# Sunshine-718/AlphaZero-AL

Hardware: AMD Instinct MI355X
Metric: self-play positions/sec (Connect4 n_playout=200, batch=8192 games/GPU, vl_batch=4) (higher is better)
Workload: dtype f32; 1 GPU; Connect4 self-play, n_playout=200, 8192 games/GPU, vl_batch=4, evaluator=cnn; c_base=1000, use_symmetry=True, lead_in_plies=12, streams_per_gpu=1, parallelism=independent game shards x1

## Files before the change

alphazero-al_amd/csrc/nn_conv.hip:

```cpp
#include <cstdio>
#include <cstdlib>

#include "az_nn.h"
#include "nn_common.h"

namespace {

constexpr int CELLS = 42, COLS = 7;
constexpr int PCOLS = 8, PCELLS = 72;
constexpr int TS = 4;
constexpr int COUT = 64;
constexpr int CELLB = 128;

template <int N>
__device__ __forceinline__ void stage_sample(const void *base, uint32_t voff, uint32_t lds_off, uint64_t last_mask)
{
    uint32_t keep;
    uint64_t ex;
    if constexpr (N == 6)
        asm volatile("s_mov_b32 %0, m0\n\ts_mov_b32 m0, %4\n\ts_nop 2\n\t"
                     "global_load_lds_dwordx4 %2, %3\n\t"
                     "global_load_lds_dwordx4 %2, %3 offset:1024\n\t"
                     "global_load_lds_dwordx4 %2, %3 offset:2048\n\t"
                     "global_load_lds_dwordx4 %2, %3 offset:3072\n\t"
                     "s_mov_b32 m0, %6\n\ts_nop 0\n\t"
                     "global_load_lds_dwordx4 %5, %3\n\t"
                     "s_and_saveexec_b64 %1, %7\n\t"
                     "global_load_lds_dwordx4 %5, %3 offset:1024\n\t"
                     "s_mov_b64 exec, %1\n\ts_mov_b32 m0, %0"
                     : "=&s"(keep), "=&s"(ex)
                     : "v"(voff), "s"(base), "s"(lds_off), "v"(voff + 4096), "s"(lds_off + 4096), "s"(last_mask)
                     : "memory", "scc");
    else
        asm volatile("s_mov_b32 %0, m0\n\ts_mov_b32 m0, %4\n\ts_nop 2\n\t"
                     "global_load_lds_dwordx4 %2, %3\n\t"
                     "global_load_lds_dwordx4 %2, %3 offset:1024\n\t"
                     "s_and_saveexec_b64 %1, %5\n\t"
                     "global_load_lds_dwordx4 %2, %3 offset:2048\n\t"
                     "s_mov_b64 exec, %1\n\ts_mov_b32 m0, %0"
                     : "=&s"(keep), "=&s"(ex)
                     : "v"(voff), "s"(base), "s"(lds_off), "s"(last_mask)
                     : "memory", "scc");
}
__device__ __forceinline__ uint32_t lds_addr(const void *p)
{
    return static_cast<uint32_t>(reinterpret_cast<uintptr_t>((__attribute__((address_space(3))) const void *)p));
}
__device__ __forceinline__ void lds_barrier()
{
    asm volatile("s_waitcnt lgkmcnt(0)" ::: "memory");
    __builtin_amdgcn_s_barrier();
    asm volatile("" ::: "memory");
}

__device__ unsigned long long g_prof[2048 * 8];

struct EmbedIn {
    const float    *features;
    const uint16_t *emb_own, *emb_opp;
    const uint16_t *pos;
    const int32_t  *gather;
    const uint64_t *bb_p1, *bb_p2;
    const int32_t  *turn, *sym;
};

struct StemIn {
    const uint64_t *bb_p1, *bb_p2;
    const int32_t  *turn, *sym;
    const int32_t  *gather;
    const uint16_t *wfrag;
    const float    *pmap;
};
constexpr int PROWS = 48, PROW = 68;
constexpr int PMAPB = PROWS * PROW * 4, FRAGB = 2 * 4 * 64 * 16;

template <int CIN, bool NORM, bool RESID, bool EMBED = false>
__global__ void __launch_bounds__(256, 2) k_conv_block(const uint16_t *x, const uint16_t *w, const uint16_t *bias,
                                                       const uint16_t *gamma, const uint16_t *beta, uint16_t *y,
                                                       int64_t B, float eps, int dbg, const int64_t *batch_dev, EmbedIn em)
{
    constexpr bool STEM = false, CHAINED = false;
    const StemIn st{};
#include "nn_conv_body.h"
}

__global__ void __launch_bounds__(256, 2) k_stem_conv_block(StemIn st, const uint16_t *w, const uint16_t *bias,
                                                            const uint16_t *gamma, const uint16_t *beta, uint16_t *y,
                                                            int64_t B, float eps, int dbg, const int64_t *batch_dev)
{
    constexpr int CIN = 64;
    constexpr bool NORM = true, RESID = true, EMBED = false, STEM = true, CHAINED = false;
    const uint16_t *x = nullptr;
    const EmbedIn em{};
#include "nn_conv_body.h"
}

struct ChainIn {
    const uint16_t *w[AZ_NN_MAX_BLOCKS], *bias[AZ_NN_MAX_BLOCKS], *gamma[AZ_NN_MAX_BLOCKS], *beta[AZ_NN_MAX_BLOCKS];
    uint16_t *y[AZ_NN_MAX_BLOCKS];
    int n;
};

__device__ __forceinline__ void layer_switch()
{
    asm volatile("s_waitcnt vmcnt(0)" ::: "memory");
    __builtin_amdgcn_fence(__ATOMIC_ACQUIRE, "agent");
    __syncthreads();
}

__global__ void __launch_bounds__(256, 2) k_conv_chain(StemIn st_in, ChainIn ch, int64_t B, float eps, int dbg, const int64_t *batch_dev_in)
{
    constexpr int CIN = 64;
    constexpr bool NORM = true, RESID = true, EMBED = false;
    const EmbedIn em{};
    {
        constexpr bool STEM = true, CHAINED = false;
        const StemIn &st = st_in;
        const uint16_t *x = nullptr, *w = ch.w[0], *bias = ch.bias[0], *gamma = ch.gamma[0], *beta = ch.beta[0];
        uint16_t *y = ch.y[0];
        const int64_t *batch_dev = batch_dev_in;
#include "nn_conv_body.h"
    }
#pragma unroll 1
    for (int layer = 1; layer < ch.n; ++layer) {
        layer_switch();
        constexpr bool STEM = false, CHAINED = true;
        const StemIn st{};
        const uint16_t *x = ch.y[layer - 1], *w = ch.w[layer], *bias = ch.bias[layer], *gamma = ch.gamma[layer], *beta = ch.beta[layer];
        uint16_t *y = ch.y[layer];
        const int64_t *batch_dev = nullptr;
#include "nn_conv_body.h"
    }
}

int g_dbg = 0;

int prepare(DeviceSetup &setup, const void *kern, size_t smem, int c_in, int64_t B, unsigned &grid, int &dbg)
{
    if (setup.cus({kern}, static_cast<int>(smem), [&] {
            if (getenv("AZ_NN_VERBOSE") != nullptr) {
                int per_cu = 0;
                (void)hipOccupancyMaxActiveBlocksPerMultiprocessor(&per_cu, kern, 256, smem);
                if (c_in < 0)
                    fprintf(stderr, "[az_nn] stem + conv chain: %zu B LDS, %d workgroups per CU\n", smem, per_cu);
                else if (c_in != 0)
                    fprintf(stderr, "[az_nn] conv block C_in=%d: %zu B LDS, %d workgroups per CU\n", c_in, smem, per_cu);
                else
                    fprintf(stderr, "[az_nn] stem + conv block: %zu B LDS, %d workgroups per CU\n", smem, per_cu);
            }
        }) == 0)
        return 2;
    static const int prio = [] { const char *e = getenv("AZ_NN_CONV_PRIO"); const int v = e ? atoi(e) : 1; return v < 0 || v > 3 ? 1 : v; }();
    const int64_t ntiles = (B + TS - 1) / TS;
    static const int64_t max_grid = getenv("AZ_NN_CONV_GRID") ? atoll(getenv("AZ_NN_CONV_GRID")) : 512;
    grid = static_cast<unsigned>(ntiles < max_grid ? ntiles : max_grid);
    dbg = (g_dbg & 255) | (((g_dbg >> 5) & 3) ? 0 : (prio << 5));
    return 0;
}

template <int CIN, bool NORM, bool RESID, bool EMBED = false>
int launch(const void *x, const void *w, const void *bias, const void *gamma, const void *beta, void *y, int64_t B,
           float eps, const int64_t *batch_dev, hipStream_t s, EmbedIn em = EmbedIn{})
{
    constexpr size_t smem = static_cast<size_t>(TS) * PCELLS * CELLB + 2 * static_cast<size_t>(TS) * CELLS * CIN * 2 +
                            (RESID ? 0 : static_cast<size_t>(TS) * CELLS * COUT * 2) + 2 * CIN * sizeof(float) + 512;
    auto kern = k_conv_block<CIN, NORM, RESID, EMBED>;
    static DeviceSetup setup;
    unsigned grid;
    int dbg;
    if (prepare(setup, reinterpret_cast<const void *>(kern), smem, CIN, B, grid, dbg) != 0) return 2;
    hipLaunchKernelGGL(kern, dim3(grid), dim3(256), smem, s, static_cast<const uint16_t *>(x),
                       static_cast<const uint16_t *>(w), static_cast<const uint16_t *>(bias),
                       static_cast<const uint16_t *>(gamma), static_cast<const uint16_t *>(beta),
                       static_cast<uint16_t *>(y), B, eps, dbg, batch_dev, em);
    return 0;
}

int launch_stem(const StemIn &st, const void *w, const void *bias, const void *gamma, const void *beta, void *y, int64_t B,
                float eps, const int64_t *batch_dev, hipStream_t s)
{
    constexpr size_t smem = static_cast<size_t>(TS) * PCELLS * CELLB + static_cast<size_t>(TS) * CELLS * 64 * 2 +
                            2 * 64 * sizeof(float) + 512 + PMAPB + FRAGB;
    static_assert(2 * smem <= 160 * 1024, "two workgroups per CU");
    static DeviceSetup setup;
    unsigned grid;
    int dbg;
    if (prepare(setup, reinterpret_cast<const void *>(k_stem_conv_block), smem, 0, B, grid, dbg) != 0) return 2;
    hipLaunchKernelGGL(k_stem_conv_block, dim3(grid), dim3(256), smem, s, st, static_cast<const uint16_t *>(w),
                       static_cast<const uint16_t *>(bias), static_cast<const uint16_t *>(gamma),
                       static_cast<const uint16_t *>(beta), static_cast<uint16_t *>(y), B, eps, dbg, batch_dev);
    return 0;
}

int launch_chain(const StemIn &st, const ChainIn &ch, int64_t B, float eps, const int64_t *batch_dev, hipStream_t s)
{
    constexpr size_t smem_block = static_cast<size_t>(TS) * PCELLS * CELLB + 2 * static_cast<size_t>(TS) * CELLS * 64 * 2 +
                                  2 * 64 * sizeof(float) + 512;
    constexpr size_t smem_stem = static_cast<size_t>(TS) * PCELLS * CELLB + static_cast<size_t>(TS) * CELLS * 64 * 2 +
                                 2 * 64 * sizeof(float) + 512 + PMAPB + FRAGB;
    constexpr size_t smem = smem_block > smem_stem ? smem_block : smem_stem;
    static_assert(smem == 80896 && 2 * smem <= 160 * 1024, "two workgroups per CU");
    static DeviceSetup setup;
    unsigned grid;
    int dbg;
    if (prepare(setup, reinterpret_cast<const void *>(k_conv_chain), smem, -1, B, grid, dbg) != 0) return 2;
    hipLaunchKernelGGL(k_conv_chain, dim3(grid), dim3(256), smem, s, st, ch, B, eps, dbg, batch_dev);
    return 0;
}

}

extern "C" {

int az_nn_debug(int flags) { g_dbg = flags; return 0; }
int az_nn_debug_flags(void) { return g_dbg; }

int az_nn_conv_profile(unsigned long long *out, int n)
{
    if (n > 2048 * 8) n = 2048 * 8;
    return hipMemcpyFromSymbol(out, HIP_SYMBOL(g_prof), sizeof(unsigned long long) * n) == hipSuccess ? 0 : 2;
}

int az_nn_conv_block(const void *x, int c_in, const void *weight_ohwi, const void *bias, const void *gamma,
                     const void *beta, int residual, void *y, int64_t batch, float eps, const int64_t *batch_dev,
                     void *stream)
{
    if (batch <= 0) return 1;
    hipStream_t s = static_cast<hipStream_t>(stream);
    const bool norm = gamma != nullptr && beta != nullptr;
    if (c_in == 64 && norm && residual) return launch<64, true, true>(x, weight_ohwi, bias, gamma, beta, y, batch, eps, batch_dev, s);
    if (c_in == 64 && norm && !residual) return launch<64, true, false>(x, weight_ohwi, bias, gamma, beta, y, batch, eps, batch_dev, s);
    if (c_in == 32 && !norm && !residual) return launch<32, false, false>(x, weight_ohwi, bias, gamma, beta, y, batch, eps, batch_dev, s);
    return 1;
}

int az_nn_stem_conv_block_positions(const az_nn_positions *positions, const void *w_frag, const float *pmap,
                                    const void *weight_ohwi, const void *bias, const void *gamma, const void *beta, void *y,
                                    int64_t batch, float eps, const int32_t *gather, const int64_t *batch_dev, void *stream)
{
    if (batch <= 0 || positions == nullptr || !positions->bb_p1 || !positions->bb_p2 || !positions->turn || !positions->sym ||
        w_frag == nullptr || pmap == nullptr || weight_ohwi == nullptr || bias == nullptr || gamma == nullptr || beta == nullptr ||
        y == nullptr)
        return 1;
    const StemIn st{positions->bb_p1, positions->bb_p2, positions->turn, positions->sym, gather,
                    static_cast<const uint16_t *>(w_frag), pmap};
    return launch_stem(st, weight_ohwi, bias, gamma, beta, y, batch, eps, batch_dev, static_cast<hipStream_t>(stream));
}

int az_nn_stem_conv_chain_positions(const az_nn_positions *positions, const void *w_frag, const float *pmap, int n_blocks,
                                    const void *const *weight_ohwi, const void *const *bias, const void *const *gamma,
                                    const void *const *beta, void *y_even, void *y_odd, int64_t batch, float eps,
                                    const int32_t *gather, const int64_t *batch_dev, void *stream)
{
    if (batch <= 0 || positions == nullptr || !positions->bb_p1 || !positions->bb_p2 || !positions->turn || !positions->sym ||
        w_frag == nullptr || pmap == nullptr || n_blocks < 1 || n_blocks > AZ_NN_MAX_BLOCKS || weight_ohwi == nullptr ||
        bias == nullptr || gamma == nullptr || beta == nullptr || y_even == nullptr || y_odd == nullptr || y_even == y_odd)
        return 1;
    ChainIn ch{};
    for (int i = 0; i < n_blocks; ++i) {
        if (!weight_ohwi[i] || !bias[i] || !gamma[i] || !beta[i]) return 1;
        ch.w[i] = static_cast<const uint16_t *>(weight_ohwi[i]);
        ch.bias[i] = static_cast<const uint16_t *>(bias[i]);
        ch.gamma[i] = static_cast<const uint16_t *>(gamma[i]);
        ch.beta[i] = static_cast<const uint16_t *>(beta[i]);
        ch.y[i] = static_cast<uint16_t *>((i & 1) ? y_odd : y_even);
    }
    ch.n = n_blocks;
    const StemIn st{positions->bb_p1, positions->bb_p2, positions->turn, positions->sym, gather,
                    static_cast<const uint16_t *>(w_frag), pmap};
    return launch_chain(st, ch, batch, eps, batch_dev, static_cast<hipStream_t>(stream));
}

int az_nn_stem_embed(const float *features, const void *emb_own, const void *emb_opp, const void *pos,
                     const void *weight_ohwi, const void *bias, void *y, int64_t batch, const int32_t *gather,
                     const int64_t *batch_dev, void *stream)
{
    if (batch <= 0 || features == nullptr) return 1;
    EmbedIn em{features, static_cast<const uint16_t *>(emb_own), static_cast<const uint16_t *>(emb_opp),
               static_cast<const uint16_t *>(pos), gather, nullptr, nullptr, nullptr, nullptr};
    return launch<32, false, false, true>(nullptr, weight_ohwi, bias, nullptr, nullptr, y, batch, 0.0f, batch_dev,
                                          static_cast<hipStream_t>(stream), em);
}

int az_nn_stem_embed_positions(const az_nn_positions *positions, const void *emb_own, const void *emb_opp, const void *pos,
                               const void *weight_ohwi, const void *bias, void *y, int64_t batch, const int32_t *gather,
                               const int64_t *batch_dev, void *stream)
{
    if (batch <= 0 || positions == nullptr || !positions->bb_p1 || !positions->bb_p2 || !positions->turn || !positions->sym) return 1;
    EmbedIn em{nullptr, static_cast<const uint16_t *>(emb_own), static_cast<const uint16_t *>(emb_opp),
               static_cast<const uint16_t *>(pos), gather, positions->bb_p1, positions->bb_p2, positions->turn, positions->sym};
    return launch<32, false, false, true>(nullptr, weight_ohwi, bias, nullptr, nullptr, y, batch, 0.0f, batch_dev,
                                          static_cast<hipStream_t>(stream), em);
}

}
```

alphazero-al_amd/csrc/nn_conv_body.h:

```cpp
    static_assert(!EMBED || (CIN == 32 && !NORM && !RESID), "the embedding is fused into the stem only");
    static_assert(!STEM || (CIN == 64 && NORM && RESID && !EMBED), "the folded stem is fused into the first residual block only");
    constexpr int NRAW = STEM ? 1 : 2;
    const int64_t rows_total = B;
    if (batch_dev != nullptr && *batch_dev < B) B = *batch_dev;
    constexpr int K = 9 * CIN;
    constexpr int KSTEPS = K / 32;
    constexpr int KPT = CIN / 32;
    constexpr int VPC = CIN / 8;
    constexpr int VPS = CELLS * VPC;
    constexpr int PER = (VPS + 63) / 64;
    constexpr int SB = VPS * 16;
    constexpr int OVPS = CELLS * COUT / 8;
    constexpr int OPER = (OVPS + 63) / 64;
    constexpr int OSB = OVPS * 16;
    constexpr int LASTN = VPS - 64 * (PER - 1), OLASTN = OVPS - 64 * (OPER - 1);
    static_assert(LASTN > 0 && LASTN < 64 && OLASTN > 0 && OLASTN < 64 && (PER == 6 || PER == 3), "stage_sample's two forms");

    extern __shared__ __align__(16) uint8_t smem[];
    uint8_t *img = smem;
    uint8_t *rawb = smem + TS * PCELLS * CELLB;
    uint8_t *outs = rawb + NRAW * TS * SB;
    float *s_gam = reinterpret_cast<float *>(outs + (RESID ? 0 : TS * OSB)), *s_bet = s_gam + CIN;
    uint8_t *dump = reinterpret_cast<uint8_t *>(s_gam + 2 * CIN);
    uint8_t *s_pm = dump + 512, *s_fr = s_pm + PMAPB;

    int tid = threadIdx.x;
    if (CHAINED) asm volatile("" : "+v"(tid));
    const int lane = tid & 63;
    const int wave = __builtin_amdgcn_readfirstlane(tid >> 6);
    const int mh = wave & 1, th = wave >> 1;
    const int l15 = lane & 15, l4 = lane >> 4;

    bf16x8 aw[2][KSTEPS];
    float bia[2][4];
#pragma unroll
    for (int mt = 0; mt < 2; ++mt) {
        const int o = mh * 32 + (l15 >> 2) * 8 + mt * 4 + (l15 & 3);
#pragma unroll
        for (int s = 0; s < KSTEPS; ++s)
            aw[mt][s] = *reinterpret_cast<const bf16x8 *>(w + static_cast<size_t>(o) * K + s * 32 + l4 * 8);
#pragma unroll
        for (int r = 0; r < 4; ++r)
            bia[mt][r] = __uint_as_float(static_cast<uint32_t>(bias[mh * 32 + l4 * 8 + mt * 4 + r]) << 16);
    }
    if (NORM && tid < CIN) {
        s_gam[tid] = __uint_as_float(static_cast<uint32_t>(gamma[tid]) << 16);
        s_bet[tid] = __uint_as_float(static_cast<uint32_t>(beta[tid]) << 16);
    }
    {
        V8 z; z.w[0] = z.w[1] = z.w[2] = z.w[3] = 0;
        constexpr int NV = (TS * PCELLS * CELLB + NRAW * TS * SB) / 16;
        for (int i = tid; i < NV; i += 256) reinterpret_cast<V8 *>(smem)[i] = z;
    }
    if (STEM) {
        for (int i = tid; i < PMAPB / 16; i += 256) reinterpret_cast<V8 *>(s_pm)[i] = reinterpret_cast<const V8 *>(st.pmap)[i];
        for (int i = tid; i < FRAGB / 16; i += 256) reinterpret_cast<V8 *>(s_fr)[i] = reinterpret_cast<const V8 *>(st.wfrag)[i];
    }
    __syncthreads();

    auto swz_in = [](int cell) { return VPC == 8 ? (cell & 7) : 0; };
    auto tok_off = [](uint32_t l, int vpc) { return vpc == 8 ? ((l >> 3) << 7) | (((l & 7) ^ ((l >> 3) & 7)) << 4) : l << 4; };
    const uint32_t raw_lds = lds_addr(rawb);
    if (EMBED) {
        for (int i = tid; i < CELLS * CIN / 8; i += 256)
            reinterpret_cast<V8 *>(rawb)[i] = reinterpret_cast<const V8 *>(em.pos)[i];
        __syncthreads();
    }
    auto stage_tile = [&](int64_t tile, int buf, uint32_t lane) {
        const int64_t b = tile * TS + wave;
        if (EMBED || STEM || b >= B) return;
        stage_sample<PER>(x + b * (CELLS * CIN), tok_off(lane, VPC), raw_lds + (buf * TS + wave) * SB, (1ull << LASTN) - 1);
    };

    const int64_t ntiles = (B + TS - 1) / TS;
    float pl_own[PER], pl_opp[PER];
    auto load_planes = [&](int64_t tile, uint32_t lane) {
        const int64_t b = tile * TS + wave;
        const bool live = b < B;
        int64_t row = !live ? 0 : (em.gather != nullptr ? em.gather[b] : b);
        if (row < 0 || row >= rows_total) row = 0;
        if (em.features != nullptr) {
            const float *fs = em.features + row * (3 * CELLS);
#pragma unroll
            for (int i = 0; i < PER; ++i) {
                const uint32_t s = lane + 64 * i;
                const bool ok = live && s < VPS;
                pl_own[i] = ok ? fs[s / VPC] : 0.0f;
                pl_opp[i] = ok ? fs[CELLS + s / VPC] : 0.0f;
            }
        } else {
            const bool p1 = em.turn[row] > 0, mir = em.sym[row] != 0;
            const uint64_t own = p1 ? em.bb_p1[row] : em.bb_p2[row], opp = p1 ? em.bb_p2[row] : em.bb_p1[row];
#pragma unroll
            for (int i = 0; i < PER; ++i) {
                const uint32_t s = lane + 64 * i;
                const bool ok = live && s < VPS;
                const int cell = ok ? s / VPC : 0;
                const int r = cell / COLS, c = cell - r * COLS;
                const int bit = (mir ? COLS - 1 - c : c) * 7 + (5 - r);
                pl_own[i] = (ok && ((own >> bit) & 1ull)) ? 1.0f : 0.0f;
                pl_opp[i] = (ok && ((opp >> bit) & 1ull)) ? 1.0f : 0.0f;
            }
        }
    };
    auto request_row = [&](int64_t tile) {
        const int64_t b = tile * TS + wave;
        int32_t r = 0;
        if (tile < ntiles && b < B && st.gather != nullptr) r = st.gather[b];
        return r;
    };
    auto request_pos = [&](int64_t tile, int32_t rowv, uint32_t lane) {
        const int64_t b = tile * TS + wave;
        uint32_t v = 0;
        if (tile < ntiles && b < B) {
            int64_t row = st.gather != nullptr ? static_cast<int64_t>(__builtin_amdgcn_readfirstlane(rowv)) : b;
            if (row < 0 || row >= rows_total) row = 0;
            const uint32_t *p1 = reinterpret_cast<const uint32_t *>(st.bb_p1 + row), *p2 = reinterpret_cast<const uint32_t *>(st.bb_p2 + row);
            const uint32_t *src = lane < 2 ? p1 + lane
                                : lane < 4 ? p2 + (lane - 2)
                                : lane == 4 ? reinterpret_cast<const uint32_t *>(st.turn + row) : reinterpret_cast<const uint32_t *>(st.sym + row);
            if (lane < 6) v = *src;
        }
        return v;
    };
    int32_t rowv = 0;
    uint32_t posv = 0;
    if (STEM) {
        rowv = request_row(blockIdx.x);
        posv = request_pos(blockIdx.x, rowv, lane);
        rowv = request_row(static_cast<int64_t>(blockIdx.x) + gridDim.x);
    }
    if (EMBED && static_cast<int64_t>(blockIdx.x) < ntiles) load_planes(blockIdx.x, lane);
    if (static_cast<int64_t>(blockIdx.x) < ntiles) stage_tile(blockIdx.x, 0, lane);
    asm volatile("s_waitcnt vmcnt(0)" ::: "memory");
    lds_barrier();
    int par = 0;
    const bool prof = dbg & 16;
    unsigned long long tp[7] = {0, 0, 0, 0, 0, 0, 0}, tl = prof ? __builtin_amdgcn_s_memtime() : 0;
    auto stamp = [&](int k) {
        if (prof) {
            const unsigned long long now = __builtin_amdgcn_s_memtime();
            tp[k] += now - tl;
            tl = now;
        }
    };
    uint32_t img_off[PER];
#pragma unroll
    for (int i = 0; i < PER; ++i) {
        const int sl = lane + 64 * i;
        const int cell = sl / VPC;
        const int r = cell / COLS, c = cell - r * COLS;
        const int p = (r + 1) * PCOLS + (c + 1);
        const int ck = (lane % VPC) ^ swz_in(lane / VPC);
        img_off[i] = static_cast<uint32_t>((wave * PCELLS + p) * CELLB + ((ck ^ (p & 7)) << 4));
    }
    for (int64_t tile = blockIdx.x; tile < ntiles; tile += gridDim.x, par ^= 1) {
        const int64_t b0 = tile * TS;
        uint8_t *rawt = rawb + (STEM ? 0 : par) * TS * SB;
        uint8_t *outt = RESID ? rawt : outs;
        int lane_o = lane;
        asm volatile("" : "+v"(lane_o));
        const uint32_t lane_t = static_cast<uint32_t>(lane_o) & 63u;

        if (STEM) {
            const uint32_t w0 = __builtin_amdgcn_readlane(posv, 0), w1 = __builtin_amdgcn_readlane(posv, 1);
            const uint32_t w2 = __builtin_amdgcn_readlane(posv, 2), w3 = __builtin_amdgcn_readlane(posv, 3);
            const bool p1 = static_cast<int32_t>(__builtin_amdgcn_readlane(posv, 4)) > 0, mir = __builtin_amdgcn_readlane(posv, 5) != 0;
            if (b0 + wave < B) {
                const uint64_t bb1 = (static_cast<uint64_t>(w1) << 32) | w0, bb2 = (static_cast<uint64_t>(w3) << 32) | w2;
                const uint64_t own = p1 ? bb1 : bb2, opp = p1 ? bb2 : bb1;
                const int g = lane_t >> 4, tl = lane_t & 15;
                const int my_r = lane_t / COLS, my_c = static_cast<int>(lane_t) - my_r * COLS;
                const int bit = (mir ? COLS - 1 - my_c : my_c) * 7 + (5 - my_r);
                const bool own_here = lane_t < CELLS && ((own >> bit) & 1ull);
                const bool opp_here = lane_t < CELLS && ((opp >> bit) & 1ull);
                const uint64_t om8 = __ballot(own_here) << 8, pm8 = __ballot(opp_here) << 8;
                int sh[4];
#pragma unroll
                for (int j = 0; j < 4; ++j) {
                    const int tp4 = g * 4 + j;
                    sh[j] = tp4 < 9 ? (tp4 / 3) * 7 + tp4 % 3 : 31;
                }
                bf16x8 bq[3];
                int tok[3];
#pragma unroll
                for (int tt = 0; tt < 3; ++tt) {
                    const int token = tt * 16 + tl;
                    tok[tt] = token;
                    const int c = token % COLS;
                    uint32_t m = 0x1C387u;
                    if (c == 0) m &= ~0x4081u;
                    if (c == COLS - 1) m &= ~0x10204u;
                    const uint32_t cmask = token < CELLS ? m : 0u;
                    const uint32_t wo = static_cast<uint32_t>(om8 >> token) & cmask;
                    const uint32_t wp = static_cast<uint32_t>(pm8 >> token) & cmask;
                    uint32_t d[4];
#pragma unroll
                    for (int j = 0; j < 4; ++j)
                        d[j] = (((wo >> sh[j]) & 1u) | (((wp >> sh[j]) & 1u) << 16)) * 0x3F80u;
                    bq[tt] = __builtin_bit_cast(bf16x8, uint4{d[0], d[1], d[2], d[3]});
                }
                const float *s_p = reinterpret_cast<const float *>(s_pm);
#pragma unroll
                for (int m = 0; m < 2; ++m) {
                    const bf16x8 h0 = *reinterpret_cast<const bf16x8 *>(s_fr + ((0 * 4 + 2 * m) * 64 + lane_t) * 16);
                    const bf16x8 h1 = *reinterpret_cast<const bf16x8 *>(s_fr + ((0 * 4 + 2 * m + 1) * 64 + lane_t) * 16);
                    const bf16x8 l0 = *reinterpret_cast<const bf16x8 *>(s_fr + ((1 * 4 + 2 * m) * 64 + lane_t) * 16);
                    const bf16x8 l1 = *reinterpret_cast<const bf16x8 *>(s_fr + ((1 * 4 + 2 * m + 1) * 64 + lane_t) * 16);
                    const int ch = m * 32 + g * 8;
#pragma unroll
                    for (int tt = 0; tt < 3; ++tt) {
                        f32x4 a0 = *reinterpret_cast<const f32x4 *>(&s_p[tok[tt] * PROW + ch]);
                        f32x4 a1 = *reinterpret_cast<const f32x4 *>(&s_p[tok[tt] * PROW + ch + 4]);
                        a0 = MFMA32(h0, bq[tt], a0);
                        a1 = MFMA32(h1, bq[tt], a1);
                        a0 = MFMA32(l0, bq[tt], a0);
                        a1 = MFMA32(l1, bq[tt], a1);
                        const f32x2 s0 = silu2(f32x2{a0[0], a0[1]}), s1 = silu2(f32x2{a0[2], a0[3]});
                        const f32x2 s2 = silu2(f32x2{a1[0], a1[1]}), s3 = silu2(f32x2{a1[2], a1[3]});
                        V8 o;
                        o.w[0] = pack2(s0.x, s0.y); o.w[1] = pack2(s1.x, s1.y); o.w[2] = pack2(s2.x, s2.y); o.w[3] = pack2(s3.x, s3.y);
                        if (tt < 2 || tok[tt] < CELLS)
                            *reinterpret_cast<V8 *>(rawt + wave * SB + tok[tt] * 128 + (((4 * m + g) ^ (tok[tt] & 7)) << 4)) = o;
                    }
                }
            }
            stamp(6);
        }
        {
            const int ck = (lane_t % VPC) ^ swz_in(lane_t / VPC);
            const bool last_ok = lane_t < LASTN;
            const uint8_t *rawl = rawt + wave * SB + lane_t * 16;
            V8 raw[PER];
            if (EMBED) {
                const V8 eo = *reinterpret_cast<const V8 *>(em.emb_own + ck * 8), ep = *reinterpret_cast<const V8 *>(em.emb_opp + ck * 8);
#pragma unroll
                for (int i = 0; i < PER; ++i) {
                    if (i < PER - 1 || last_ok) {
                        const V8 ps = *reinterpret_cast<const V8 *>(rawb + lane_t * 16 + i * 1024);
                        const f32x2 own = {pl_own[i], pl_own[i]}, opp = {pl_opp[i], pl_opp[i]};
#pragma unroll
                        for (int q = 0; q < 4; ++q) {
                            const f32x2 v = unpack2(ps.w[q]) + own * unpack2(eo.w[q]) + opp * unpack2(ep.w[q]);
                            raw[i].w[q] = pack2(v.x, v.y);
                        }
                    } else {
                        raw[i].w[0] = raw[i].w[1] = raw[i].w[2] = raw[i].w[3] = 0;
                    }
                }
            } else {
#pragma unroll
                for (int i = 0; i < PER; ++i) {
                    if (i < PER - 1 || last_ok) raw[i] = *reinterpret_cast<const V8 *>(rawl + i * 1024);
                    else raw[i].w[0] = raw[i].w[1] = raw[i].w[2] = raw[i].w[3] = 0;
                }
            }
            f32x2 sc[4], sh[4];
            if (NORM) {
                f32x2 sum2 = {0.0f, 0.0f}, sq2 = {0.0f, 0.0f};
#pragma unroll
                for (int i = 0; i < PER; ++i) {
#pragma unroll
                    for (int q = 0; q < 4; ++q) {
                        const f32x2 f = unpack2(raw[i].w[q]);
                        sum2 += f;
                        sq2 = __builtin_elementwise_fma(f, f, sq2);
                    }
                }
                const float sum = wave_sum(sum2.x + sum2.y), sq = wave_sum(sq2.x + sq2.y);
                const float mean = sum * (1.0f / (CELLS * CIN));
                const float var = fmaxf(sq * (1.0f / (CELLS * CIN)) - mean * mean, 0.0f);
                const float rstd = rsqrtf(var + eps);
#pragma unroll
                for (int q = 0; q < 4; ++q) {
                    const f32x2 gq = *reinterpret_cast<const f32x2 *>(&s_gam[ck * 8 + 2 * q]);
                    const f32x2 bq = *reinterpret_cast<const f32x2 *>(&s_bet[ck * 8 + 2 * q]);
                    sc[q] = gq * f32x2{rstd, rstd};
                    sh[q] = bq - sc[q] * f32x2{mean, mean};
                }
            }
#pragma unroll
            for (int i = 0; i < PER; ++i) {
                if (i < PER - 1 || last_ok) {
                    V8 out = raw[i];
                    if (NORM) {
#pragma unroll
                        for (int q = 0; q < 4; ++q) {
                            const f32x2 f = __builtin_elementwise_fma(unpack2(raw[i].w[q]), sc[q], sh[q]);
                            out.w[q] = pack2(f.x, f.y);
                        }
                    }
                    *reinterpret_cast<V8 *>(img + img_off[i]) = out;
                }
            }
        }
        stamp(0);
        lds_barrier();
        stamp(1);
        if (tile + gridDim.x < ntiles) {
            stage_tile(tile + gridDim.x, par ^ 1, lane_t);
            if (EMBED) load_planes(tile + gridDim.x, lane_t);
        }
        if (STEM) {
            posv = request_pos(tile + gridDim.x, rowv, lane_t);
            rowv = request_row(tile + 2 * static_cast<int64_t>(gridDim.x));
        }

        uint32_t col[3][KPT];
        {
            const uint32_t pc = static_cast<uint32_t>(2 * th * PCELLS + l15 + 9 - PCOLS - 1);
#pragma unroll
            for (int d = 0; d < 3; ++d) {
                const uint32_t p = pc + d;
                const uint32_t o = (p * CELLB + ((l4 ^ (p & 7)) << 4)) & 0xffffu;
#pragma unroll
                for (int ks = 0; ks < KPT; ++ks) col[d][ks] = o ^ (ks << 6);
            }
        }
        auto fetch = [&](int it, int tap, bf16x8 (&xf)[KPT]) {
            const int dy = tap / 3, d = tap % 3;
            const int disp = (dy * PCOLS + (it / 3) * PCELLS + (it % 3) * 16) * CELLB;
#pragma unroll
            for (int ks = 0; ks < KPT; ++ks)
                xf[ks] = *reinterpret_cast<const bf16x8 *>(&smem[col[d][ks] + disp]);
        };
        struct Epi { V8 *slot; V8 rr, o; f32x2 t, v; };
        auto epi_begin = [&](int it, Epi &e) {
            const int smp = 2 * th + it / 3, t = (it % 3) * 16 + l15;
            const int cell = (t >> 3) * COLS + (t & 7);
            const uint32_t m = (t & 7) == 7 ? 0xffffffffu : 0u;
            const uint32_t off_real = static_cast<uint32_t>(outt - smem) + smp * OSB + cell * 128 + (((mh * 4 + l4) ^ (cell & 7)) << 4);
            const uint32_t off_dump = static_cast<uint32_t>(dump - smem) + (wave * 8 + (l15 >> 3) + 2 * l4) * 16;
            e.slot = reinterpret_cast<V8 *>(&smem[(off_real & ~m) | (off_dump & m)]);
            if (RESID) e.rr = *e.slot;
        };
        auto epi_step = [&](int step, const f32x4 (&acc)[2], Epi &e) {
            const int q = step / 9;
            const f32x2 x = {acc[q >> 1][2 * (q & 1)], acc[q >> 1][2 * (q & 1) + 1]};
            switch (step % 9) {
            case 0: e.t = x * f32x2{-1.44269504f, -1.44269504f}; break;
            case 1: e.t.x = __builtin_amdgcn_exp2f(e.t.x); break;
            case 2: e.t.y = __builtin_amdgcn_exp2f(e.t.y); break;
            case 3: e.t += f32x2{1.0f, 1.0f}; break;
            case 4: e.t.x = __builtin_amdgcn_rcpf(e.t.x); break;
            case 5: e.t.y = __builtin_amdgcn_rcpf(e.t.y); break;
            case 6: e.v = x * e.t; break;
            case 7: if (RESID) e.v += unpack2(e.rr.w[q]); break;
            default: e.o.w[q] = pack2(e.v.x, e.v.y); break;
            }
        };
        auto epi_end = [&](Epi &e) { *e.slot = e.o; };

        auto block = [&](int it, f32x4 (&acc)[2], bool with_epi, const f32x4 (&pacc)[2]) {
#pragma unroll
            for (int mt = 0; mt < 2; ++mt) acc[mt] = f32x4{bia[mt][0], bia[mt][1], bia[mt][2], bia[mt][3]};
            Epi e;
            if (with_epi) epi_begin(it - 1, e);
            bf16x8 xa[KPT], xb[KPT];
            fetch(it, 0, xa);
            __builtin_amdgcn_sched_barrier(0);
#pragma unroll
            for (int tap = 0; tap < 9; ++tap) {
                bf16x8 (&cur)[KPT] = (tap & 1) ? xb : xa;
                bf16x8 (&nxt)[KPT] = (tap & 1) ? xa : xb;
                if (tap + 1 < 9) fetch(it, tap + 1, nxt);
                __builtin_amdgcn_sched_barrier(0);
#pragma unroll
                for (int ks = 0; ks < KPT; ++ks)
#pragma unroll
                    for (int mt = 0; mt < 2; ++mt) {
                        const int s = tap * KPT + ks;
                        acc[mt] = __builtin_amdgcn_mfma_f32_16x16x32_bf16(aw[mt][s], cur[ks], acc[mt], 0, 0, 0);
                        if (with_epi) {
                            __builtin_amdgcn_sched_barrier(0);
                            constexpr int PER_SLOT = 36 / (18 * KPT);
                            const int slot = (tap * KPT + ks) * 2 + mt;
#pragma unroll
                            for (int j = 0; j < PER_SLOT; ++j) epi_step(slot * PER_SLOT + j, pacc, e);
                            __builtin_amdgcn_sched_barrier(0);
                        }
                    }
            }
            if (with_epi) epi_end(e);
        };
        if (!(dbg & 1)) {
            if ((dbg >> 5) & 3) {
                if (((dbg >> 5) & 3) == 1) __builtin_amdgcn_s_setprio(1);
                else if (((dbg >> 5) & 3) == 2) __builtin_amdgcn_s_setprio(2);
                else __builtin_amdgcn_s_setprio(3);
            }
            f32x4 acc_a[2], acc_b[2];
            block(0, acc_a, false, acc_b);
            block(1, acc_b, true, acc_a);
            block(2, acc_a, true, acc_b);
            block(3, acc_b, true, acc_a);
            block(4, acc_a, true, acc_b);
            block(5, acc_b, true, acc_a);
            {
                Epi e;
                epi_begin(5, e);
#pragma unroll
                for (int step = 0; step < 36; ++step) epi_step(step, acc_b, e);
                epi_end(e);
            }
            if ((dbg >> 5) & 3) __builtin_amdgcn_s_setprio(0);
        }
        stamp(2);
        asm volatile("s_waitcnt vmcnt(0)" ::: "memory");
        stamp(3);
        lds_barrier();
        stamp(4);

        if (b0 + wave < B && !(dbg & 2)) {
            constexpr int MID = (OPER / 2) * 1024;
            uint8_t *ym = reinterpret_cast<uint8_t *>(y + (b0 + wave) * (CELLS * COUT)) + MID;
            uint32_t outl = static_cast<uint32_t>(outt - smem) + wave * OSB + lane_t * 16;
            asm volatile("" : "+s"(ym), "+v"(outl));
            auto *ymg = (__attribute__((address_space(1))) uint8_t *)ym;
            const uint32_t yo = tok_off(lane_t, COUT / 8);
#pragma unroll
            for (int i = 0; i < OPER; ++i) {
                if (i < OPER - 1 || lane_t < OLASTN) {
                    const V8 v = *reinterpret_cast<const V8 *>(&smem[outl + i * 1024]);
                    *reinterpret_cast<__attribute__((address_space(1))) f32x4 *>(ymg + yo + (i * 1024 - MID)) = __builtin_bit_cast(f32x4, v);
                }
            }
        }
        stamp(5);
    }
    if (prof && lane == 0 && blockIdx.x < 512)
        for (int k = 0; k < (STEM ? 7 : 6); ++k) g_prof[(blockIdx.x * 4 + wave) * 8 + k] = tp[k];
```

Before: 310,400 positions/s.

## Serpentine tile order across chained conv layers and drop per-layer barrier

In the chained conv kernel, odd layers now walk each block's tiles in reverse. A block therefore starts each layer on the tile it just finished, whose residual output is still in its LDS raw buffer, so the initial restage and wait are skipped. The full vmcnt wait, agent-scope acquire fence and __syncthreads between layers become a single `buffer_inv sc1` cache invalidate. This relies on every block consuming only tiles it produced itself. Weight, bias, gamma/beta and stem-table global loads are also issued before the LDS zeroing and barrier to hide their latency, and optional profiling marks are added.

```diff
diff --git a/alphazero-al_amd/csrc/nn_conv.hip b/alphazero-al_amd/csrc/nn_conv.hip
--- a/alphazero-al_amd/csrc/nn_conv.hip
+++ b/alphazero-al_amd/csrc/nn_conv.hip
@@ -54,6 +54,21 @@
 }
 
 __device__ unsigned long long g_prof[2048 * 8];
+enum ProfMark { MARK_ENTRY, MARK_FIRST_TILE, MARK_LAYER_END, MARK_LAYER_FIRST_TILE };
+__device__ __forceinline__ void prof_mark(ProfMark what)
+{
+    if ((threadIdx.x & 63) != 0 || blockIdx.x >= 512) return;
+    unsigned long long *slot = g_prof + (blockIdx.x * 4 + (threadIdx.x >> 6)) * 8 + 7;
+    const unsigned long long lo = 0xffffffffull, now = __builtin_amdgcn_s_memtime() & lo, v = *slot;
+    *slot = what == MARK_ENTRY        ? now
+#ifdef AZ_CONV_PROF_ENTRY
+          : what == MARK_FIRST_TILE   ? ((now - v) & lo) << 32
+#else
+          : what == MARK_FIRST_TILE   ? 0
+#endif
+          : what == MARK_LAYER_END    ? (v & ~lo) | ((v - now) & lo)
+                                      : (v & ~lo) | ((v + now) & lo);
+}
 
 struct EmbedIn {
     const float    *features;
@@ -71,16 +86,29 @@
     const uint16_t *wfrag;
     const float    *pmap;
 };
+struct Carry {
+    int64_t tile;
+    int par;
+};
 constexpr int PROWS = 48, PROW = 68;
 constexpr int PMAPB = PROWS * PROW * 4, FRAGB = 2 * 4 * 64 * 16;
+
+__device__ __forceinline__ void layer_switch()
+{
+    asm volatile("buffer_inv sc1" ::: "memory");
+}
 
 template <int CIN, bool NORM, bool RESID, bool EMBED = false>
 __global__ void __launch_bounds__(256, 2) k_conv_block(const uint16_t *x, const uint16_t *w, const uint16_t *bias,
                                                        const uint16_t *gamma, const uint16_t *beta, uint16_t *y,
                                                        int64_t B, float eps, int dbg, const int64_t *batch_dev, EmbedIn em)
 {
-    constexpr bool STEM = false, CHAINED = false;
+    constexpr bool STEM = false, CHAINED = false, desc = false;
     const StemIn st{};
+    Carry carry{0, 0};
+#ifdef AZ_CONV_PROF_ENTRY
+    if (dbg & 16) prof_mark(MARK_ENTRY);
+#endif
 #include "nn_conv_body.h"
 }
 
@@ -90,8 +118,13 @@
 {
     constexpr int CIN = 64;
     constexpr bool NORM = true, RESID = true, EMBED = false, STEM = true, CHAINED = false;
+    constexpr bool desc = false;
     const uint16_t *x = nullptr;
     const EmbedIn em{};
+    Carry carry{0, 0};
+#ifdef AZ_CONV_PROF_ENTRY
+    if (dbg & 16) prof_mark(MARK_ENTRY);
+#endif
 #include "nn_conv_body.h"
 }
 
@@ -101,20 +134,17 @@
     int n;
 };
 
-__device__ __forceinline__ void layer_switch()
-{
-    asm volatile("s_waitcnt vmcnt(0)" ::: "memory");
-    __builtin_amdgcn_fence(__ATOMIC_ACQUIRE, "agent");
-    __syncthreads();
-}
-
 __global__ void __launch_bounds__(256, 2) k_conv_chain(StemIn st_in, ChainIn ch, int64_t B, float eps, int dbg, const int64_t *batch_dev_in)
 {
     constexpr int CIN = 64;
     constexpr bool NORM = true, RESID = true, EMBED = false;
     const EmbedIn em{};
+    Carry carry{0, 0};
+#ifdef AZ_CONV_PROF_ENTRY
+    if (dbg & 16) prof_mark(MARK_ENTRY);
+#endif
     {
-        constexpr bool STEM = true, CHAINED = false;
+        constexpr bool STEM = true, CHAINED = false, desc = false;
         const StemIn &st = st_in;
         const uint16_t *x = nullptr, *w = ch.w[0], *bias = ch.bias[0], *gamma = ch.gamma[0], *beta = ch.beta[0];
         uint16_t *y = ch.y[0];
@@ -123,8 +153,9 @@
     }
 #pragma unroll 1
     for (int layer = 1; layer < ch.n; ++layer) {
-        layer_switch();
+        if (dbg & 16) prof_mark(MARK_LAYER_END);
         constexpr bool STEM = false, CHAINED = true;
+        const bool desc = layer & 1;
         const StemIn st{};
         const uint16_t *x = ch.y[layer - 1], *w = ch.w[layer], *bias = ch.bias[layer], *gamma = ch.gamma[layer], *beta = ch.beta[layer];
         uint16_t *y = ch.y[layer];
diff --git a/alphazero-al_amd/csrc/nn_conv_body.h b/alphazero-al_amd/csrc/nn_conv_body.h
--- a/alphazero-al_amd/csrc/nn_conv_body.h
+++ b/alphazero-al_amd/csrc/nn_conv_body.h
@@ -31,78 +31,7 @@
     const int mh = wave & 1, th = wave >> 1;
     const int l15 = lane & 15, l4 = lane >> 4;
 
-    bf16x8 aw[2][KSTEPS];
-    float bia[2][4];
-#pragma unroll
-    for (int mt = 0; mt < 2; ++mt) {
-        const int o = mh * 32 + (l15 >> 2) * 8 + mt * 4 + (l15 & 3);
-#pragma unroll
-        for (int s = 0; s < KSTEPS; ++s)
-            aw[mt][s] = *reinterpret_cast<const bf16x8 *>(w + static_cast<size_t>(o) * K + s * 32 + l4 * 8);
-#pragma unroll
-        for (int r = 0; r < 4; ++r)
-            bia[mt][r] = __uint_as_float(static_cast<uint32_t>(bias[mh * 32 + l4 * 8 + mt * 4 + r]) << 16);
-    }
-    if (NORM && tid < CIN) {
-        s_gam[tid] = __uint_as_float(static_cast<uint32_t>(gamma[tid]) << 16);
-        s_bet[tid] = __uint_as_float(static_cast<uint32_t>(beta[tid]) << 16);
-    }
-    {
-        V8 z; z.w[0] = z.w[1] = z.w[2] = z.w[3] = 0;
-        constexpr int NV = (TS * PCELLS * CELLB + NRAW * TS * SB) / 16;
-        for (int i = tid; i < NV; i += 256) reinterpret_cast<V8 *>(smem)[i] = z;
-    }
-    if (STEM) {
-        for (int i = tid; i < PMAPB / 16; i += 256) reinterpret_cast<V8 *>(s_pm)[i] = reinterpret_cast<const V8 *>(st.pmap)[i];
-        for (int i = tid; i < FRAGB / 16; i += 256) reinterpret_cast<V8 *>(s_fr)[i] = reinterpret_cast<const V8 *>(st.wfrag)[i];
-    }
-    __syncthreads();
-
-    auto swz_in = [](int cell) { return VPC == 8 ? (cell & 7) : 0; };
-    auto tok_off = [](uint32_t l, int vpc) { return vpc == 8 ? ((l >> 3) << 7) | (((l & 7) ^ ((l >> 3) & 7)) << 4) : l << 4; };
-    const uint32_t raw_lds = lds_addr(rawb);
-    if (EMBED) {
-        for (int i = tid; i < CELLS * CIN / 8; i += 256)
-            reinterpret_cast<V8 *>(rawb)[i] = reinterpret_cast<const V8 *>(em.pos)[i];
-        __syncthreads();
-    }
-    auto stage_tile = [&](int64_t tile, int buf, uint32_t lane) {
-        const int64_t b = tile * TS + wave;
-        if (EMBED || STEM || b >= B) return;
-        stage_sample<PER>(x + b * (CELLS * CIN), tok_off(lane, VPC), raw_lds + (buf * TS + wave) * SB, (1ull << LASTN) - 1);
-    };
-
     const int64_t ntiles = (B + TS - 1) / TS;
-    float pl_own[PER], pl_opp[PER];
-    auto load_planes = [&](int64_t tile, uint32_t lane) {
-        const int64_t b = tile * TS + wave;
-        const bool live = b < B;
-        int64_t row = !live ? 0 : (em.gather != nullptr ? em.gather[b] : b);
-        if (row < 0 || row >= rows_total) row = 0;
-        if (em.features != nullptr) {
-            const float *fs = em.features + row * (3 * CELLS);
-#pragma unroll
-            for (int i = 0; i < PER; ++i) {
-                const uint32_t s = lane + 64 * i;
-                const bool ok = live && s < VPS;
-                pl_own[i] = ok ? fs[s / VPC] : 0.0f;
-                pl_opp[i] = ok ? fs[CELLS + s / VPC] : 0.0f;
-            }
-        } else {
-            const bool p1 = em.turn[row] > 0, mir = em.sym[row] != 0;
-            const uint64_t own = p1 ? em.bb_p1[row] : em.bb_p2[row], opp = p1 ? em.bb_p2[row] : em.bb_p1[row];
-#pragma unroll
-            for (int i = 0; i < PER; ++i) {
-                const uint32_t s = lane + 64 * i;
-                const bool ok = live && s < VPS;
-                const int cell = ok ? s / VPC : 0;
-                const int r = cell / COLS, c = cell - r * COLS;
-                const int bit = (mir ? COLS - 1 - c : c) * 7 + (5 - r);
-                pl_own[i] = (ok && ((own >> bit) & 1ull)) ? 1.0f : 0.0f;
-                pl_opp[i] = (ok && ((opp >> bit) & 1ull)) ? 1.0f : 0.0f;
-            }
-        }
-    };
     auto request_row = [&](int64_t tile) {
         const int64_t b = tile * TS + wave;
         int32_t r = 0;
@@ -125,18 +54,115 @@
     };
     int32_t rowv = 0;
     uint32_t posv = 0;
+
+    constexpr int NTAB = (PMAPB + FRAGB) / 16, TPER = (NTAB + 255) / 256;
+    f32x4 tab[TPER];
     if (STEM) {
         rowv = request_row(blockIdx.x);
+#pragma unroll
+        for (int j = 0; j < TPER; ++j) {
+            const int i = tid + 256 * j < NTAB ? tid + 256 * j : NTAB - 1;
+            tab[j] = i < PMAPB / 16 ? reinterpret_cast<const f32x4 *>(st.pmap)[i] : reinterpret_cast<const f32x4 *>(st.wfrag)[i - PMAPB / 16];
+        }
+    }
+    uint16_t gam_b = 0, bet_b = 0;
+    if (NORM) {
+        gam_b = gamma[tid & (CIN - 1)];
+        bet_b = beta[tid & (CIN - 1)];
+    }
+    asm volatile("" ::: "memory");
+    bf16x8 aw[2][KSTEPS];
+    float bia[2][4];
+#pragma unroll
+    for (int mt = 0; mt < 2; ++mt) {
+        const int o = mh * 32 + (l15 >> 2) * 8 + mt * 4 + (l15 & 3);
+#pragma unroll
+        for (int s = 0; s < KSTEPS; ++s)
+            aw[mt][s] = *reinterpret_cast<const bf16x8 *>(w + static_cast<size_t>(o) * K + s * 32 + l4 * 8);
+#pragma unroll
+        for (int r = 0; r < 4; ++r)
+            bia[mt][r] = __uint_as_float(static_cast<uint32_t>(bias[mh * 32 + l4 * 8 + mt * 4 + r]) << 16);
+    }
+    if (CHAINED) layer_switch();
+    if (STEM) {
         posv = request_pos(blockIdx.x, rowv, lane);
         rowv = request_row(static_cast<int64_t>(blockIdx.x) + gridDim.x);
     }
+    asm volatile("" ::: "memory");
+    if (!CHAINED) {
+        V8 z; z.w[0] = z.w[1] = z.w[2] = z.w[3] = 0;
+        constexpr int NV = (TS * PCELLS * CELLB + NRAW * TS * SB) / 16;
+        for (int i = tid; i < NV; i += 256) reinterpret_cast<V8 *>(smem)[i] = z;
+    }
+    if (STEM) {
+#pragma unroll
+        for (int j = 0; j < TPER; ++j)
+            if (tid + 256 * j < NTAB) reinterpret_cast<f32x4 *>(s_pm)[tid + 256 * j] = tab[j];
+    }
+    if (NORM) {
+        s_gam[tid & (CIN - 1)] = __uint_as_float(static_cast<uint32_t>(gam_b) << 16);
+        s_bet[tid & (CIN - 1)] = __uint_as_float(static_cast<uint32_t>(bet_b) << 16);
+    }
+    if (CHAINED) lds_barrier();
+    else __syncthreads();
+
+    auto swz_in = [](int cell) { return VPC == 8 ? (cell & 7) : 0; };
+    auto tok_off = [](uint32_t l, int vpc) { return vpc == 8 ? ((l >> 3) << 7) | (((l & 7) ^ ((l >> 3) & 7)) << 4) : l << 4; };
+    const uint32_t raw_lds = lds_addr(rawb);
+    if (EMBED) {
+        for (int i = tid; i < CELLS * CIN / 8; i += 256)
+            reinterpret_cast<V8 *>(rawb)[i] = reinterpret_cast<const V8 *>(em.pos)[i];
+        __syncthreads();
+    }
+    auto stage_tile = [&](int64_t tile, int buf, uint32_t lane) {
+        const int64_t b = tile * TS + wave;
+        if (EMBED || STEM || b >= B) return;
+        stage_sample<PER>(x + b * (CELLS * CIN), tok_off(lane, VPC), raw_lds + (buf * TS + wave) * SB, (1ull << LASTN) - 1);
+    };
+
+    float pl_own[PER], pl_opp[PER];
+    auto load_planes = [&](int64_t tile, uint32_t lane) {
+        const int64_t b = tile * TS + wave;
+        const bool live = b < B;
+        int64_t row = !live ? 0 : (em.gather != nullptr ? em.gather[b] : b);
+        if (row < 0 || row >= rows_total) row = 0;
+        if (em.features != nullptr) {
+            const float *fs = em.features + row * (3 * CELLS);
+#pragma unroll
+            for (int i = 0; i < PER; ++i) {
+                const uint32_t s = lane + 64 * i;
+                const bool ok = live && s < VPS;
+                pl_own[i] = ok ? fs[s / VPC] : 0.0f;
+                pl_opp[i] = ok ? fs[CELLS + s / VPC] : 0.0f;
+            }
+        } else {
+            const bool p1 = em.turn[row] > 0, mir = em.sym[row] != 0;
+            const uint64_t own = p1 ? em.bb_p1[row] : em.bb_p2[row], opp = p1 ? em.bb_p2[row] : em.bb_p1[row];
+#pragma unroll
+            for (int i = 0; i < PER; ++i) {
+                const uint32_t s = lane + 64 * i;
+                const bool ok = live && s < VPS;
+                const int cell = ok ? s / VPC : 0;
+                const int r = cell / COLS, c = cell - r * COLS;
+                const int bit = (mir ? COLS - 1 - c : c) * 7 + (5 - r);
+                pl_own[i] = (ok && ((own >> bit) & 1ull)) ? 1.0f : 0.0f;
+                pl_opp[i] = (ok && ((opp >> bit) & 1ull)) ? 1.0f : 0.0f;
+            }
+        }
+    };
     if (EMBED && static_cast<int64_t>(blockIdx.x) < ntiles) load_planes(blockIdx.x, lane);
-    if (static_cast<int64_t>(blockIdx.x) < ntiles) stage_tile(blockIdx.x, 0, lane);
-    asm volatile("s_waitcnt vmcnt(0)" ::: "memory");
-    lds_barrier();
-    int par = 0;
+    const int64_t tstep = (CHAINED && desc) ? -static_cast<int64_t>(gridDim.x) : static_cast<int64_t>(gridDim.x);
+    auto is_tile = [&](int64_t t) { return CHAINED ? static_cast<uint64_t>(t) < static_cast<uint64_t>(ntiles) : t < ntiles; };
+    int64_t tile = (CHAINED && desc) ? carry.tile : static_cast<int64_t>(blockIdx.x);
+    int par = CHAINED ? carry.par : 0;
+    if (!CHAINED) {
+        if (is_tile(tile)) stage_tile(tile, 0, lane);
+        asm volatile("s_waitcnt vmcnt(0)" ::: "memory");
+        lds_barrier();
+    }
     const bool prof = dbg & 16;
     unsigned long long tp[7] = {0, 0, 0, 0, 0, 0, 0}, tl = prof ? __builtin_amdgcn_s_memtime() : 0;
+    if (prof) prof_mark(CHAINED ? MARK_LAYER_FIRST_TILE : MARK_FIRST_TILE);
     auto stamp = [&](int k) {
         if (prof) {
             const unsigned long long now = __builtin_amdgcn_s_memtime();
@@ -154,7 +180,7 @@
         const int ck = (lane % VPC) ^ swz_in(lane / VPC);
         img_off[i] = static_cast<uint32_t>((wave * PCELLS + p) * CELLB + ((ck ^ (p & 7)) << 4));
     }
-    for (int64_t tile = blockIdx.x; tile < ntiles; tile += gridDim.x, par ^= 1) {
+    for (; is_tile(tile); tile += tstep, par ^= 1) {
         const int64_t b0 = tile * TS;
         uint8_t *rawt = rawb + (STEM ? 0 : par) * TS * SB;
         uint8_t *outt = RESID ? rawt : outs;
@@ -297,9 +323,9 @@
         stamp(0);
         lds_barrier();
         stamp(1);
-        if (tile + gridDim.x < ntiles) {
-            stage_tile(tile + gridDim.x, par ^ 1, lane_t);
-            if (EMBED) load_planes(tile + gridDim.x, lane_t);
+        if (is_tile(tile + tstep)) {
+            stage_tile(tile + tstep, par ^ 1, lane_t);
+            if (EMBED) load_planes(tile + tstep, lane_t);
         }
         if (STEM) {
             posv = request_pos(tile + gridDim.x, rowv, lane_t);
@@ -428,5 +454,9 @@
         }
         stamp(5);
     }
-    if (prof && lane == 0 && blockIdx.x < 512)
-        for (int k = 0; k < (STEM ? 7 : 6); ++k) g_prof[(blockIdx.x * 4 + wave) * 8 + k] = tp[k];
+    carry.tile = tile - tstep;
+    carry.par = STEM ? 0 : par ^ 1;
+    if (prof && lane == 0 && blockIdx.x < 512) {
+        unsigned long long *row = g_prof + (blockIdx.x * 4 + wave) * 8;
+        for (int k = 0; k < (STEM ? 7 : 6); ++k) row[k] = CHAINED ? row[k] + tp[k] : tp[k];
+    }
```

Result: no change. 311,600 positions/s (median of 6 runs) (+0.4%).
